# SegoleneMartin/transductive-CLIP

Hardware: AMD Instinct MI355X
Metric: transductive tasks/sec (75-query EM-Dirichlet) (higher is better)
Workload: dtype f32

## Files before the change

### transductive-clip_amd/csrc/tclip_device.h

```cpp
#pragma once
#include <hip/hip_runtime.h>

#include "tclip_math.h"
#include "tclip_rsqrt14_table_dev.h"

namespace tclip {

constexpr int kGroup = 32;
constexpr float kEpsF = 1e-15f;

template <int N>
__device__ __forceinline__ float dpp_row_shl(float v) {
    static_assert(N >= 1 && N <= 15, "row_shl");
    return __builtin_bit_cast(float, __builtin_amdgcn_update_dpp(0, __builtin_bit_cast(int, v), 0x100 + N, 0xf, 0xf, true));
}
__device__ __forceinline__ float ordered_sum8_lane0(float fin, float p0) {
    fin += p0;
    fin += dpp_row_shl<1>(p0);
    fin += dpp_row_shl<2>(p0);
    fin += dpp_row_shl<3>(p0);
    fin += dpp_row_shl<4>(p0);
    fin += dpp_row_shl<5>(p0);
    fin += dpp_row_shl<6>(p0);
    fin += dpp_row_shl<7>(p0);
// ... 254 lines not shown
    const float big = __builtin_fabsf(div_rn_inrange_f32(2.0f * t, a * a));
    const float curv = (a > 1e-11f) ? big : 1.6449340668482264f;
    float b = (psi1 - psi_s) - curv * a;
    b = b - y;
    const float delta = b * b + 4.0f * curv;
    const float nume = -b + sqrt_torch_inrange_dev(delta), deno = 2.0f * curv;
    return deno == 0.0f ? nume * __builtin_inff() : div_rn_inrange_f32(nume, deno);
}

__device__ __forceinline__ float mm_update(float a, float y, float psi_s, const LogTabEntry* tab) {
    float psi1, lg1;
    digamma_lgamma_xp1(a, tab, psi1, lg1);
    return mm_update_algebra(a, y, psi_s, psi1, lg1);
}

__device__ __noinline__ float mm_update_generic(float a, float y, float psi_s) {
    const float x1 = a + 1.0f;
    const float psi1 = digamma_f32(x1);
    const float lg1 = lgamma_f32(x1);
    float curv;
    if (a > 1e-11f) {
        const float t = (0.0f - lg1) + psi1 * a;
        curv = __builtin_fabsf((2.0f * t) / (a * a));
    } else {
        curv = 1.6449340668482264f;
    }
    float b = (psi1 - psi_s) - curv * a;
    b = b - y;
    const float delta = b * b + 4.0f * curv;
    return (-b + sqrt_torch_f32(delta)) / (2.0f * curv);
}

__device__ __forceinline__ void load_log_table(LogTabEntry* lds_tab) {
    if (threadIdx.x < 16) lds_tab[threadIdx.x] = kLogTab[threadIdx.x];
    __syncthreads();
}

}
```

### transductive-clip_amd/csrc/tclip_kernels.hip

```cpp
#include <hip/hip_runtime.h>
#include <stdint.h>
#include <stdio.h>
#include <stdlib.h>
#include <string.h>

#include <algorithm>
#include <mutex>
#include <utility>
#include <vector>

#include "../../include/tclip.h"
#include "tclip_device.h"
#include "tclip_pk.h"
#include "tclip_selftest_inputs.h"

namespace tclip {

constexpr int kG64MinK = 897;

__global__ void k_log_features(const float* __restrict__ x, float* __restrict__ out, size_t n, int32_t* __restrict__ nonfinite) {
    bool bad = false;
    for (size_t i = (size_t)blockIdx.x * blockDim.x + threadIdx.x; i < n; i += (size_t)gridDim.x * blockDim.x) {
        const float v = log_f32(x[i] + kEpsF);
        out[i] = v;
// ... 571 lines not shown
    }
    const float psi_s = digamma_pos_f32(s, tab);
    int n_big = 0;
#pragma unroll
    for (int e = 0; e < E; e++) {
        const float x1 = beta[e] + 1.0f;
        const bool big = x1 >= 2.3f;
        const unsigned long long m = __ballot(big);
        if (big) queue[n_big + lanes_below(m)] = x1;
        n_big += __popcll(m);
    }
    __builtin_amdgcn_wave_barrier();
    const unsigned long long active = __ballot(true);
    const int rank = lanes_below(active), n_active = __popcll(active);
    for (int start = 0; start < n_big; start += n_active) {
        const int idx = start + rank;
        const float v = idx < n_big ? queue[idx] : 8.0f;
        const float r = lgamma_big_dense(v);
        if (idx < n_big) queue[idx] = r;
    }
    __builtin_amdgcn_wave_barrier();
    if (n_big == 0) mm_apply_updates_small<E, G>(beta, yv, K, lane, psi_s, tab, measure, num, den);
    else mm_apply_updates<E, G>(beta, yv, K, lane, psi_s, tab, queue, 0, measure, num, den);
    __builtin_amdgcn_wave_barrier();
}

constexpr int kProbeChunks = 2;
constexpr int kMaxCycle = 64;

constexpr int kMMWavesLarge = 3;
constexpr int kMMWavesSmall = 4;
template <int E, int G>
__global__ __launch_bounds__(256, (E > 16 ? kMMWavesLarge : kMMWavesSmall)) void k_mm_probe(MMArgs a) {
    __shared__ LogTabEntry tab[16];
    __shared__ double cyc[256 / G][kMaxCycle][2];
    __shared__ float lg_queue[4][64 * E];
    load_log_table(tab);
    float* queue = lg_queue[threadIdx.x >> 6];
    const int lane = threadIdx.x & (G - 1);
    const int group = threadIdx.x / G;
    const int groups_per_block = blockDim.x / G;
    const int n = *a.n_rows;
    const int K = a.K;
    for (int i = blockIdx.x * groups_per_block + group; i < n; i += gridDim.x * groups_per_block) {
        const int row = a.rows[i];
        if (a.stop[row / a.rows_per_batch]) continue;
        const int have = a.cache_len[row];
        if (have != a.chunk + 1) {
            if (a.next_rows && have < a.n_checks && lane == 0) a.next_rows[atomicAdd(a.next_count, 1)] = row;
            continue;
        }
        const float* ref = a.beta_dead + (size_t)row * K;
        float beta[E];
        RowY<E, G> yv;
        yv.load(nullptr, lane, K);
#pragma unroll
        for (int e = 0; e < E; e++) {
            const int d = elem_of<E, G>(e, lane);
            beta[e] = d < K ? ref[d] : 0.0f;
        }
        int period = 0;
        for (int j = 0; j < kMaxCycle && period == 0; j++) {
            double pn = 0.0, pd = 0.0;
            mm_iterate<E, G>(beta, yv, K, lane, tab, queue, true, pn, pd);
            pn = group_sum_f64_g<G>(pn);
            pd = group_sum_f64_g<G>(pd);
            if (lane == 0) { cyc[group][j][0] = pn; cyc[group][j][1] = pd; }
            bool same = true;
#pragma unroll
            for (int e = 0; e < E; e++) {
                const int d = elem_of<E, G>(e, lane);
                if (d < K) same = same && (beta[e] == ref[d]);
            }
            const unsigned long long bal = __ballot(same);
            constexpr unsigned long long kAll = G == 64 ? ~0ull : (1ull << (G & 63)) - 1ull;
            const unsigned long long mine = (bal >> ((threadIdx.x & 63) & ~(G - 1))) & kAll;
            if (mine == kAll) period = j + 1;
        }
        if (period && lane == 0) {
            for (int m = a.chunk + 1; m < a.n_checks; m++) {
                const int j = (50 * (m + 1) - (a.l1 + 1)) % period;
                double* c = a.cache + ((size_t)row * a.n_checks + m) * 2;
                c[0] = cyc[group][j][0];
                c[1] = cyc[group][j][1];
            }
            a.cache_len[row] = a.n_checks;
        }
        if (!period && a.next_rows && lane == 0) a.next_rows[atomicAdd(a.next_count, 1)] = row;
    }
}

constexpr int kDeadHead = 12;
static_assert(kDeadHead <= 18, "the last snapshot (32 iterations after the head) must lie at or before the first checkpoint (iteration 50)");
template <int E, int G>
__global__ __launch_bounds__(256, (E > 16 ? kMMWavesLarge : kMMWavesSmall)) void k_mm_probe_head(MMArgs a) {
    __shared__ LogTabEntry tab[16];
    __shared__ double cyc[256 / G][kMaxCycle][2];
    __shared__ float lg_queue[4][64 * E];
    load_log_table(tab);
    float* queue = lg_queue[threadIdx.x >> 6];
    const int lane = threadIdx.x & (G - 1);
    const int group = threadIdx.x / G;
    const int groups_per_block = blockDim.x / G;
    const int n = *a.n_rows;
    const int K = a.K;
    for (int i = blockIdx.x * groups_per_block + group; i < n; i += gridDim.x * groups_per_block) {
        const int row = a.rows[i];
        if (a.stop[row / a.rows_per_batch]) continue;
        if (a.cache_len[row] != 0) {
            if (lane == 0) a.next_rows[atomicAdd(a.next_count, 1)] = row;
            continue;
        }
        float* ref = a.beta_dead + (size_t)row * K;
        float* ref8 = const_cast<float*>(a.y) + (size_t)row * K;
        float beta[E];
        RowY<E, G> yv;
        yv.load(nullptr, lane, K);
#pragma unroll
        for (int e = 0; e < E; e++) {
            const int d = elem_of<E, G>(e, lane);
            beta[e] = d < K ? ref[d] : 0.0f;
        }
        int period = 0, js = 0, base = 0;
        bool have8 = false;
        constexpr unsigned long long kAll = G == 64 ? ~0ull : (1ull << (G & 63)) - 1ull;
        const int shift = (threadIdx.x & 63) & ~(G - 1);
        for (int j = 0; j < kMaxCycle && period == 0; j++) {
            double pn = 0.0, pd = 0.0;
            mm_iterate<E, G>(beta, yv, K, lane, tab, queue, true, pn, pd);
// ... 121 lines not shown
        }
        __syncthreads();
        return;
    }
    for (int start = ((wave + turn) % W) * 64; start < n_big; start += 64 * W) {
        const int j = start + lane64;
        int at = j;
#pragma unroll
        for (int w = 1; w < W; w++) at += j >= before[w] ? 64 * E * R - (before[w] - before[w - 1]) : 0;
        const float v = j < n_big ? queue[at] : 8.0f;
        const float r = lgamma_big_dense(v);
        if (j < n_big) queue[at] = r;
    }
    if (wave == (W - (turn % W) + 1) % W && lane64 < kGroups * R)
        ctl->psi[turn & 1][lane64] = digamma_pos_f32(ctl->rowsum[turn & 1][lane64], tab);
    __syncthreads();
    if (base[R] == 0) {
#pragma unroll
        for (int r = 0; r < R; r++)
            if (active[r])
                mm_apply_updates_small<E, G>(beta[r], yv[r], K, lane, ctl->psi[turn & 1][r * kGroups + (threadIdx.x / G)], tab,
                                             measure, num[r], den[r]);
        return;
    }
#pragma unroll
    for (int r = 0; r < R; r++)
        if (active[r])
            mm_apply_updates<E, G>(beta[r], yv[r], K, lane, ctl->psi[turn & 1][r * kGroups + (threadIdx.x / G)], tab, slice, base[r],
                                   measure, num[r], den[r]);
}

template <int E, int W, bool kDead, int R, int G = kGroup, int KC = 0>
__global__ __launch_bounds__(64 * W, (E > 16 ? kMMWavesLarge : kMMWavesSmall)) void k_mm_live(MMArgs a) {
    __shared__ LogTabEntry tab[16];
    __shared__ float queue[64 * W * E * R];
    __shared__ QueueCtl ctl;
    if (threadIdx.x == 0) ctl.bad = 0;
    load_log_table(tab);
    const int lane = threadIdx.x & (G - 1);
    const int group = threadIdx.x / G;
    constexpr int kGroups = (64 / G) * W, kRows = kGroups * R;
    static_assert(kRows <= 64, "QueueCtl holds 64 row sums");
    int turn = 0;
    const int n = *a.n_rows;
    const int K = KC > 0 ? KC : a.K;
    for (int first = blockIdx.x * kRows; first < n; first += gridDim.x * kRows) {
        int row[R];
        bool active[R];
        bool any = false;
#pragma unroll
        for (int r = 0; r < R; r++) {
            const int i = first + r * kGroups + group;
            row[r] = i < n ? a.rows[i] : 0;
            if constexpr (G == 64) row[r] = __builtin_amdgcn_readfirstlane(row[r]);
            const bool running = i < n && !a.stop[row[r] / a.rows_per_batch];
            const int have = (kDead && running) ? a.cache_len[row[r]] : 0;
            active[r] = running && (!kDead || have == a.chunk);
            any = any || active[r];
            if (kDead && a.next_rows && running && have < a.n_checks && lane == 0)
                a.next_rows[atomicAdd(a.next_count, 1)] = row[r];
        }
        if (!__syncthreads_or(any)) continue;
        const float* src = (kDead && a.chunk > 0) ? a.beta_dead : a.alpha;
        float* dst = kDead ? a.beta_dead : a.alpha;
        float beta[R][E];
        RowY<E, G> yv[R];
        double num[R], den[R];
// ... 199 lines not shown
        uint32_t largest = 0u;
#pragma unroll
        for (int e = 0; e < E; e++) largest = max(largest, f32_bits(beta[e]));
        in_domain = in_domain & mm_fast_domain_of_max_bits(largest);
    }
    s = __shfl(s, 0, G);
    if (__builtin_expect(!__all(in_domain), 0)) {
        if (active) {
            const float psi_s = digamma_f32(s);
#pragma unroll
            for (int e = 0; e < E; e++) {
                const float nb = mm_update_generic(beta[e], yv.get(e), psi_s);
                const bool ok = elem_of<E, G>(e, lane) < K;
                if (measure && ok) {
                    const double df = (double)nb - (double)beta[e];
                    num += df * df;
                    den += (double)beta[e] * (double)beta[e];
                }
                beta[e] = ok ? nb : 0.0f;
            }
        }
        pl.valid = false;
        return;
    }
    constexpr int kFirstRagged = first_ragged_register<E, G, KC>();
    int32_t smallest = 0x7f800000;
#pragma unroll
    for (int e = 0; e < E; e++) {
        int32_t bits = (int32_t)f32_bits(beta[e]);
        if (e >= kFirstRagged) bits = elem_of<E, G>(e, lane) < K ? bits : 0x7f800000;
        smallest = bits < smallest ? bits : smallest;
    }
    const bool tiny = __builtin_amdgcn_ballot_w64(smallest <= (int32_t)0x2d2febffu) != 0ull;
    const float psi_s = digamma_pos_f32(s, tab);
    bool sort_now = !(keep_placement && pl.valid);
    for (;;) {
        if (sort_now) {
            split_place<E, G, KC>(beta, K, lane, my0, pl);
            pl.sorts++;
        } else split_scatter<E, G, KC>(beta, K, lane, my0, pl);
        const int nA = pl.nA, nB = pl.nB, nC = pl.nC;
        wave_lds_handoff();
        bool misplaced = false;
        int jA = 0;
        for (; jA + 64 < nA; jA += 128) {
            const int j = jA;
            const int i0 = j + lane64, i1 = min(i0 + 64, nA - 1);
            const f2 x{my0[i0], my0[i1]};
            if (!sort_now && __builtin_amdgcn_ballot_w64(!(fmaxf(x.x, x.y) < 2.3f)) != 0ull) { misplaced = true; break; }
            f2 xr = x, acc = pk(0.0f);
#pragma unroll
            for (int k = 0; k < 8; k++) {
                acc = acc - pk_rcp_rn(xr);
                xr = xr + pk(1.0f);
            }
            const f2 m{below10_f32(xr.x), below10_f32(xr.y)};
            acc = pk_fma(-m, pk_rcp_rn(xr), acc);
            xr = xr + m;
            const f2 psi = pk_digamma_after_rec(xr, acc, tab);
            const f2 lg = pk_lgamma_sleef_1_23(x);
            my0[i0] = lg.x;
            my1[i0] = psi.x;
            my0[i1] = lg.y;
            my1[i1] = psi.y;
        }
        for (; !misplaced && jA < nA; jA += 64) {
            const int i = min(jA + lane64, nA - 1);
            const float x = my0[i];
            if (!sort_now && __builtin_amdgcn_ballot_w64(!(x < 2.3f)) != 0ull) { misplaced = true; break; }
            float xr = x, acc = 0.0f;
#pragma unroll
            for (int k = 0; k < 8; k++) {
                acc = acc - rcp_rn_f32(xr);
                xr = xr + 1.0f;
            }
            const float m = below10_f32(xr);
            acc = __builtin_fmaf(-m, rcp_rn_f32(xr), acc);
            xr = xr + m;
            const float psi = digamma_after_rec_ge10<false>(xr, acc, tab);
            bool sure;
            float lg = lgamma_sleef_1_23_f64(x, sure);
            if (__builtin_expect(__builtin_amdgcn_ballot_w64(!sure) != 0ull, 0)) lg = sure ? lg : lgamma_sleef_05_23(x);
            my0[i] = lg;
            my1[i] = psi;
        }
        auto pass_b = [&](int i) -> bool {
            const float x = my0[i];
            if (!sort_now && __builtin_amdgcn_ballot_w64(!(x >= 2.3f)) != 0ull) return true;
            float xr = x, acc = 0.0f;
#pragma unroll
            for (int k = 0; k < 8; k++) {
                const float m = below10_f32(xr);
                acc = __builtin_fmaf(-m, rcp_rn_f32(xr), acc);
                xr += m;
            }
            const float psi = digamma_after_rec_ge10<false>(xr, acc, tab);
            const float lg = lgamma_big_dense(x);
            my0[i] = lg;
            my1[i] = psi;
            return false;
        };
        const int tB = nB & 63, tC = nC & 63;
        const bool merged = tB > 0 && tC > 0 && tB + tC <= 64;
        const int endB = merged ? nB - tB : nB, endC = merged ? nC - tC : nC;
        for (int j = 0; !misplaced && j < endB; j += 64) misplaced = pass_b(nA + min(j + lane64, endB - 1));
        if (merged && !misplaced) {
            const int l = min(lane64, tB + tC - 1);
            misplaced = pass_b(l < tB ? nA + endB + l : nA + nB + endC + (l - tB));
        }
        for (int j = 0; !misplaced && j < endC; j += 64) {
            const int i = nA + nB + min(j + lane64, endC - 1);
            const float x = my0[i];
            if (!sort_now && __builtin_amdgcn_ballot_w64(!(x >= 10.0f)) != 0ull) { misplaced = true; break; }
            const float psi = digamma_after_rec_ge10<true>(x, 0.0f, tab);
            const float lg = lgamma_gt7_dense(x);
            my0[i] = lg;
            my1[i] = psi;
        }
        if (!misplaced) break;
        sort_now = true;
        wave_lds_handoff();
    }
    pl.valid = true;
    wave_lds_handoff();
    if (__builtin_expect(measure, 0)) {
        if (tiny) split_apply_updates<E, G, true, true>(beta, yv, K, lane, psi_s, my0, my1, pl.slot, num, den);
        else split_apply_updates<E, G, false, true>(beta, yv, K, lane, psi_s, my0, my1, pl.slot, num, den);
    } else if (__builtin_expect(tiny, 0)) split_apply_updates<E, G, true, false>(beta, yv, K, lane, psi_s, my0, my1, pl.slot, num, den);
    else split_apply_updates<E, G, false, false>(beta, yv, K, lane, psi_s, my0, my1, pl.slot, num, den);
    wave_lds_handoff();
}

template <int E, int G, int KC = 0>
__global__ __launch_bounds__(64, (E > 16 ? kMMWavesLarge : kMMWavesSmall)) void k_mm_split(MMArgs a) {
    static_assert(E <= kSplitMaxE, "LDS: two words per element");
    __shared__ LogTabEntry tab[16];
    __shared__ float plane0[64 * E];
    __shared__ float plane1[64 * E];
    load_log_table(tab);
    const int lane = threadIdx.x & (G - 1);
    const int group = threadIdx.x / G;
    constexpr int kRows = 64 / G;
    const int n = *a.n_rows;
    const int K = KC > 0 ? KC : a.K;
    for (int first = blockIdx.x * kRows; first < n; first += gridDim.x * kRows) {
        const int i = first + group;
        int row = i < n ? a.rows[i] : 0;
        if constexpr (G == 64) row = __builtin_amdgcn_readfirstlane(row);
        const bool active = i < n && !a.stop[row / a.rows_per_batch];
        if (!__any(active)) continue;
        float beta[E];
        RowY<E, G, kSplitYRegsMaxE> yv;
        double num = 0.0, den = 0.0;
        yv.load(a.y + (size_t)row * K, lane, K);
#pragma unroll
        for (int e = 0; e < E; e++) {
            const int d = elem_of<E, G>(e, lane);
            beta[e] = (active && d < K) ? a.alpha[(size_t)row * K + d] : 0.0f;
        }
        SplitPlacement<E> pl;
        pl.valid = false;
        pl.sorts = 0;
        for (int l = a.l0; l <= a.l1; l++)
            mm_iterate_wave_split<E, G, KC>(beta, yv, K, lane, active, tab, plane0, plane1, a.has_check && l == a.l1, num, den, pl,
                                            a.keep_placement != 0);
        if (a.work_counter && (threadIdx.x & 63) == 0) {
            atomicAdd(a.work_counter + 1, (unsigned long long)(a.l1 - a.l0 + 1));
            atomicAdd(a.work_counter + 2, (unsigned long long)pl.sorts);
        }
// ... 989 lines not shown
                blk = 0.0f;
#pragma unroll 8
                for (int j = 0; j < kFrontBlock; j++) blk = __builtin_fmaf(emb[d + j], tr[d + j], blk);
                acc += blk;
            }
            blk = 0.0f;
            for (; d < D; d++) blk = __builtin_fmaf(emb[d], tr[d], blk);
        }
        if (full < D) acc += blk;
        if (kScaleAfter) acc = temperature * acc;
        logit[k] = acc;
        mx = acc > mx ? acc : mx;
    }
    for (int m = 32; m >= 1; m >>= 1) { const float o = __shfl_xor(mx, m, 64); mx = o > mx ? o : mx; }
    __syncthreads();
    if (lane == 0) red[4 + wave] = mx;
    __syncthreads();
    mx = fmaxf(fmaxf(red[4], red[5]), fmaxf(red[6], red[7]));
    float sum = 0.0f;
    for (int k = tid; k < K; k += blockDim.x) {
        const float e = exp_f32_sleef(logit[k] - mx);
        logit[k] = e;
        sum += e;
    }
    for (int m = 32; m >= 1; m >>= 1) sum += __shfl_xor(sum, m, 64);
    __syncthreads();
    if (lane == 0) red[wave] = sum;
    __syncthreads();
    const float inv = 1.0f / (red[0] + red[1] + red[2] + red[3]);
    for (int k = tid; k < K; k += blockDim.x) z[(size_t)n * K + k] = logit[k] * inv;
}

__global__ void k_selftest(unsigned long long* out) {
    __shared__ LogTabEntry tab[16];
    load_log_table(tab);
    const uint32_t tid = blockIdx.x * blockDim.x + threadIdx.x, nth = gridDim.x * blockDim.x;
    unsigned long long b0 = 0, b1 = 0, b2 = 0, b3 = 0, b4 = 0, b5 = 0;
    for (uint32_t m = tid; m < (1u << 23); m += nth) {
        const float x = bits_f32(0x3f800000u | m);
        b0 += rcp_rn_f32(x) != 1.0f / x;
        b5 += rcp_rn2_f32(x) != 1.0f / x;
        const float xs = x * 0x1p-60f, xl = x * 0x1p60f;
        b0 += rcp_rn_f32(xs) != 1.0f / xs;
        b0 += rcp_rn_f32(xl) != 1.0f / xl;
    }
    for (uint32_t i = tid; i < (1u << 28); i += nth) {
        const float a = rand_float(i, 1u, -40, 81), b = rand_float(i, 2u, -40, 81);
        b1 += div_rn_inrange_f32(a, b) != a / b;
        b1 += div_rn_inrange_f32(-a, b) != (-a) / b;
    }
    for (uint32_t i = tid; i < (1u << 24); i += nth) {
        const float a = rand_float(i, 3u, -45, 70);
        float p, l;
        digamma_lgamma_xp1(a, tab, p, l);
        b2 += p != digamma_f32(a + 1.0f);
        b2 += digamma_pos_f32(a, tab) != digamma_f32(a);
        b3 += l != lgamma_f32(a + 1.0f);
        const uint32_t h = mix32(i * 7u + 3u);
        const float y = -0.001f - 40.0f * (float)(h & 0xffffu) / 65536.0f;
        const float ps = 0.5f + 14.0f * (float)(h >> 16) / 65536.0f;
        const float uf = mm_update(a, y, ps, tab), ug = mm_update_generic(a, y, ps);
        const bool differ = !(uf == ug || (uf != uf && ug != ug));
        b4 += differ;
        if (differ) { out[14] = f32_bits(a); out[15] = f32_bits(y); out[16] = f32_bits(ps); out[17] = f32_bits(uf); out[18] = f32_bits(ug); }
        const float a2 = rand_float(i, 4u, -12, 18);
        const f2 av{a, a2};
        const f2 lgb{a + 1.0f >= 2.3f ? lgamma_sleef_ge23<true>(a + 1.0f) : 0.0f,
// ... 1280 lines not shown
```

### transductive-clip_amd/csrc/tclip_math.h

```cpp
#pragma once
#include <stdint.h>

#include "tclip_rsqrt14_table.h"
#include "tclip_rcp14_log_table.h"

#if defined(__HIPCC__)
#define TCLIP_HD __host__ __device__ __forceinline__
#else
#define TCLIP_HD static inline
#endif

namespace tclip {

TCLIP_HD uint32_t f32_bits(float f) { return __builtin_bit_cast(uint32_t, f); }
TCLIP_HD float bits_f32(uint32_t u) { return __builtin_bit_cast(float, u); }
TCLIP_HD uint64_t f64_bits(double f) { return __builtin_bit_cast(uint64_t, f); }
TCLIP_HD double bits_f64(uint64_t u) { return __builtin_bit_cast(double, u); }

TCLIP_HD float rcp_rn_f32(float x) {
#if defined(__HIP_DEVICE_COMPILE__)
    const float r = __builtin_amdgcn_rcpf(x);
    const float e = __builtin_fmaf(-x, r, 1.0f);
    return __builtin_fmaf(e, r, r);
#else
// ... 1 lines not shown
#endif
}

TCLIP_HD float rcp_rn2_f32(float x) {
#if defined(__HIP_DEVICE_COMPILE__)
    float r = __builtin_amdgcn_rcpf(x);
    float e = __builtin_fmaf(-x, r, 1.0f);
    r = __builtin_fmaf(e, r, r);
    e = __builtin_fmaf(-x, r, 1.0f);
    return __builtin_fmaf(e, r, r);
#else
    return 1.0f / x;
#endif
}

TCLIP_HD float div_rn_inrange_f32(float a, float b) {
#if defined(__HIP_DEVICE_COMPILE__)
    const float r = rcp_rn_f32(b);
    const float q = a * r;
    const float rem = __builtin_fmaf(-b, q, a);
    return __builtin_fmaf(rem, r, q);
#else
    return a / b;
#endif
}

template <bool kFast>
TCLIP_HD float rcp_ieee(float x) {
    if (kFast) return rcp_rn_f32(x);
    return 1.0f / x;
}

struct LogTabEntry { double invc, logc; };
#define TCLIP_LOG_TABLE_INIT { \
    {0x1.661ec79f8f3bep+0, -0x1.57bf7808caadep-2}, {0x1.571ed4aaf883dp+0, -0x1.2bef0a7c06ddbp-2}, \
    {0x1.49539f0f010bp+0, -0x1.01eae7f513a67p-2},  {0x1.3c995b0b80385p+0, -0x1.b31d8a68224e9p-3}, \
    {0x1.30d190c8864a5p+0, -0x1.6574f0ac07758p-3}, {0x1.25e227b0b8eap+0, -0x1.1aa2bc79c81p-3},   \
    {0x1.1bb4a4a1a343fp+0, -0x1.a4e76ce8c0e5ep-4}, {0x1.12358f08ae5bap+0, -0x1.1973c5a611cccp-4}, \
    {0x1.0953f419900a7p+0, -0x1.252f438e10c1ep-5}, {0x1p+0, 0x0p+0},                             \
    {0x1.e608cfd9a47acp-1, 0x1.aa5aa5df25984p-5},  {0x1.ca4b31f026aap-1, 0x1.c5e53aa362eb4p-4},   \
    {0x1.b2036576afce6p-1, 0x1.526e57720db08p-3},  {0x1.9c2d163a1aa2dp-1, 0x1.bc2860d22477p-3},   \
    {0x1.886e6037841edp-1, 0x1.1058bc8a07ee1p-2},  {0x1.767dcf5534862p-1, 0x1.4043057b6ee09p-2}}

#if defined(__HIP_DEVICE_COMPILE__)
static __device__ __constant__ LogTabEntry kLogTab[16] = TCLIP_LOG_TABLE_INIT;
#else
static const LogTabEntry kLogTab[16] = TCLIP_LOG_TABLE_INIT;
#endif

constexpr double kLn2 = 0x1.62e42fefa39efp-1;

TCLIP_HD void log_reduce_tab(float x, const LogTabEntry* tab, double& r, double& y0) {
    const uint32_t ix = f32_bits(x);
    const uint32_t tmp = ix - 0x3f330000u;
    const int i = (tmp >> 19) & 15;
    const int k = (int32_t)tmp >> 23;
    const double z = (double)bits_f32(ix - (tmp & 0xff800000u));
    const LogTabEntry t = tab[i];
    r = __builtin_fma(z, t.invc, -1.0);
    y0 = t.logc + (double)k * kLn2;
}

TCLIP_HD float logf_glibc_tab(float x, const LogTabEntry* tab) {
    if (f32_bits(x) == 0x3f800000u) return 0.0f;
    double r, y0;
    log_reduce_tab(x, tab, r, y0);
    const double r2 = r * r;
    double y = __builtin_fma(0x1.5575b0be00b6ap-2, r, -0x1.ffffef20a4123p-2);
    y = __builtin_fma(-0x1.00ea348b88334p-2, r2, y);
    y = __builtin_fma(y, r2, y0 + r);
    return (float)y;
}
TCLIP_HD float logf_glibc(float x) { return logf_glibc_tab(x, kLogTab); }

#define TCLIP_SLN_T1 {0.0f, -0x1.f800000000000p-6f, -0x1.f0c0000000000p-5f, -0x1.6f00000000000p-4f, -0x1.e280000000000p-4f, -0x1.2950000000000p-3f, -0x1.5ff0000000000p-3f, -0x1.9520000000000p-3f, -0x1.c900000000000p-3f, -0x1.fb90000000000p-3f, -0x1.1678000000000p-2f, -0x1.2e90000000000p-2f, -0x1.4618000000000p-2f, -0x1.5d18000000000p-2f, -0x1.73a0000000000p-2f, -0x1.89a0000000000p-2f, -0x1.9f30000000000p-2f, -0x1.b450000000000p-2f, -0x1.c900000000000p-2f, -0x1.dd48000000000p-2f, -0x1.f128000000000p-2f, -0x1.0254000000000p-1f, -0x1.0be8000000000p-1f, -0x1.154c000000000p-1f, -0x1.1e84000000000p-1f, -0x1.2794000000000p-1f, -0x1.307c000000000p-1f, -0x1.3940000000000p-1f, -0x1.41d8000000000p-1f, -0x1.4a50000000000p-1f, -0x1.52a4000000000p-1f, -0x1.5ad4000000000p-1f}
#define TCLIP_SLN_T2 {0.0f, -0x1.4d873c0000000p-17f, 0x1.cf3fee0000000p-17f, -0x1.a515ca0000000p-17f, 0x1.f123aa0000000p-17f, -0x1.4be0800000000p-17f, -0x1.83853c0000000p-18f, -0x1.6a73d20000000p-17f, 0x1.070cac0000000p-20f, -0x1.86d5e40000000p-19f, 0x1.1aa2a20000000p-17f, 0x1.d451ee0000000p-18f, -0x1.78438c0000000p-19f, -0x1.edfac00000000p-17f, 0x1.404a220000000p-17f, -0x1.9c360a0000000p-17f, -0x1.1f65fc0000000p-17f, 0x1.10866e0000000p-19f, 0x1.070cac0000000p-19f, 0x1.5fb3e40000000p-18f, -0x1.ebf5e00000000p-19f, -0x1.2a5a5e0000000p-17f, 0x1.a37b5a0000000p-18f, -0x1.e97a6a0000000p-20f, -0x1.f5e7040000000p-17f, -0x1.e1289c0000000p-17f, -0x1.7334f20000000p-17f, 0x1.f2ca9e0000000p-17f, -0x1.fd08ce0000000p-18f, 0x1.e893f00000000p-19f, 0x1.2d9a440000000p-17f, -0x1.30d67c0000000p-23f}
struct Rcp14Buckets { uint32_t e[64]; };
constexpr Rcp14Buckets make_rcp14_buckets() {
    constexpr uint32_t start[TCLIP_RCP14_LOG_STEPS] = TCLIP_RCP14_LOG_START;
    Rcp14Buckets b{};
    for (uint32_t q = 0; q < 64; q++) {
        const uint32_t lo = q << 17, hi = lo + (1u << 17);
        uint32_t base = 0, thr = 1u << 23;
        for (int t = 1; t < TCLIP_RCP14_LOG_STEPS; t++) {
            if (start[t] <= lo) base++;
            else if (start[t] < hi) thr = start[t];
        }
        b.e[q] = (thr << 6) | base;
    }
    return b;
}
constexpr bool rcp14_table_is_regular() {
    constexpr uint32_t start[TCLIP_RCP14_LOG_STEPS] = TCLIP_RCP14_LOG_START;
// ... 482 lines not shown
}
TCLIP_HD float digamma_rec_acc_ge23(float x1) {
    float x = x1, acc = 0.0f;
#if defined(__HIP_DEVICE_COMPILE__)
#pragma unroll
#endif
    for (int j = 0; j < 8; j++) {
        const float m = below10_f32(x);
        acc = __builtin_fmaf(-m, rcp_rn_f32(x), acc);
        x += m;
    }
    return acc;
}
TCLIP_HD float digamma_rec_x_loop(float x1) {
    float x = x1;
    for (int j = 0; j < 9; j++) x += below10_f32(x);
    return x;
}
TCLIP_HD float digamma_rec_x(float x1) {
    const float f = x1 - __builtin_floorf(x1);
    const float r8 = ((f + 2.0f) + 2.0f) + 4.0f;
#if defined(__HIP_DEVICE_COMPILE__)
    const float up = __builtin_amdgcn_fmed3f(__builtin_fmaf(r8, 0x1p20f, 1.0f - 9.0f * 0x1p20f), 0.0f, 1.0f);
#else
    const float up = r8 == 9.0f ? 1.0f : 0.0f;
#endif
    const float small_x = (r8 + 2.0f) - up;
    return x1 < 10.0f ? small_x : x1;
}
TCLIP_HD float digamma_after_rec(float x, float acc, const LogTabEntry* tab) {
    const float series = digamma_series<true>(x, acc, tab);
    return (x == 10.0f) ? acc + 2.25175258906672110764f : series;
}
template <bool kNoAcc>
TCLIP_HD float digamma_after_rec_ge10(float x, float acc, const LogTabEntry* tab) {
    const float z = rcp_ieee<true>(x * x);
    float p = 8.33333333333333333333E-2f;
    p = __builtin_fmaf(p, z, -2.10927960927960927961E-2f);
    p = __builtin_fmaf(p, z, 7.57575757575757575758E-3f);
    p = __builtin_fmaf(p, z, -4.16666666666666666667E-3f);
    p = __builtin_fmaf(p, z, 3.96825396825396825397E-3f);
    p = __builtin_fmaf(p, z, -8.33333333333333333333E-3f);
    p = __builtin_fmaf(p, z, 8.33333333333333333333E-2f);
    const float y = z * p;
    double r, y0;
    log_reduce_tab(x, tab, r, y0);
    const double r2 = r * r;
    double l = __builtin_fma(0x1.5575b0be00b6ap-2, r, -0x1.ffffef20a4123p-2);
    l = __builtin_fma(-0x1.00ea348b88334p-2, r2, l);
    l = __builtin_fma(l, r2, y0 + r);
    const float lg = (float)l;
    const float series = ((kNoAcc ? lg : acc + lg) - 0.5f * rcp_ieee<true>(x)) - y;
    const float at10 = kNoAcc ? 2.25175258906672110764f : acc + 2.25175258906672110764f;
#if defined(__HIP_DEVICE_COMPILE__)
    if (__builtin_expect(__builtin_amdgcn_ballot_w64(x == 10.0f) == 0ull, 1)) return series;
#endif
    return (x == 10.0f) ? at10 : series;
}

TCLIP_HD void digamma_lgamma_xp1(float a, const LogTabEntry* tab, float& psi1, float& lg1) {
    psi1 = digamma_xp1(a, tab);
    const float x1 = a + 1.0f;
    const bool lo = x1 < 2.3f;
    const float small_x = lgamma_sleef_05_23(lo ? x1 : 2.0f);
    const float large_x = lgamma_sleef_ge23<true>(lo ? 8.0f : x1);
    lg1 = lo ? small_x : large_x;
}

}
```

### transductive-clip_amd/csrc/tclip_pk.h

```cpp
#pragma once
#include "tclip_device.h"

namespace tclip {

typedef float f2 __attribute__((ext_vector_type(2)));
typedef int i2 __attribute__((ext_vector_type(2)));

__device__ __forceinline__ f2 pk(float v) { return f2{v, v}; }
__device__ __forceinline__ f2 pk_fma(f2 a, f2 b, f2 c) { return __builtin_elementwise_fma(a, b, c); }
__device__ __forceinline__ f2 pk_sel(i2 m, f2 a, f2 b) { return m ? a : b; }
__device__ __forceinline__ f2 pk_sel(i2 m, float a, float b) { return m ? pk(a) : pk(b); }

__device__ __forceinline__ f2 pk_rcp_rn(f2 x) {
    f2 r{__builtin_amdgcn_rcpf(x.x), __builtin_amdgcn_rcpf(x.y)};
    const f2 e = pk_fma(-x, r, pk(1.0f));
    return pk_fma(e, r, r);
}

__device__ __forceinline__ f2 pk_div_rn(f2 a, f2 b) {
    const f2 r = pk_rcp_rn(b);
    const f2 q = a * r;
    const f2 rem = pk_fma(-b, q, a);
    return pk_fma(rem, r, q);
}

__device__ __forceinline__ f2 pk_div_rn_negden(f2 a, f2 nb) {
    const f2 r0{__builtin_amdgcn_rcpf(-nb.x), __builtin_amdgcn_rcpf(-nb.y)};
    const f2 r = pk_fma(pk_fma(nb, r0, pk(1.0f)), r0, r0);
    const f2 q = a * r;
    return pk_fma(pk_fma(nb, q, a), r, q);
}

__device__ __forceinline__ f2 pk_logf_glibc_ne1(f2 x, const LogTabEntry* tab) {
    const uint32_t ix0 = f32_bits(x.x), ix1 = f32_bits(x.y);
    const uint32_t tmp0 = ix0 - 0x3f330000u, tmp1 = ix1 - 0x3f330000u;
    const LogTabEntry e0 = tab[(tmp0 >> 19) & 15], e1 = tab[(tmp1 >> 19) & 15];
    const double z0 = (double)bits_f32(ix0 - (tmp0 & 0xff800000u)), z1 = (double)bits_f32(ix1 - (tmp1 & 0xff800000u));
    const double r0 = __builtin_fma(z0, e0.invc, -1.0), r1 = __builtin_fma(z1, e1.invc, -1.0);
    const double y00 = e0.logc + (double)((int32_t)tmp0 >> 23) * kLn2, y01 = e1.logc + (double)((int32_t)tmp1 >> 23) * kLn2;
    const double q0 = r0 * r0, q1 = r1 * r1;
    double y0 = __builtin_fma(0x1.5575b0be00b6ap-2, r0, -0x1.ffffef20a4123p-2);
    double y1 = __builtin_fma(0x1.5575b0be00b6ap-2, r1, -0x1.ffffef20a4123p-2);
    y0 = __builtin_fma(-0x1.00ea348b88334p-2, q0, y0);
    y1 = __builtin_fma(-0x1.00ea348b88334p-2, q1, y1);
    y0 = __builtin_fma(y0, q0, y00 + r0);
    y1 = __builtin_fma(y1, q1, y01 + r1);
    return f2{(float)y0, (float)y1};
}

__device__ __forceinline__ f2 pk_digamma_xp1(f2 a, const LogTabEntry* tab) {
    f2 x = a + pk(1.0f), acc = pk(0.0f);
#pragma unroll
    for (int j = 0; j < 9; j++) {
        const f2 m{below10_f32(x.x), below10_f32(x.y)};
        const f2 r = pk_rcp_rn(x);
        acc = pk_fma(-m, r, acc);
        x = x + m;
    }
    const f2 z = pk_rcp_rn(x * x);
    f2 p = pk(8.33333333333333333333E-2f);
    p = pk_fma(p, z, pk(-2.10927960927960927961E-2f));
    p = pk_fma(p, z, pk(7.57575757575757575758E-3f));
    p = pk_fma(p, z, pk(-4.16666666666666666667E-3f));
    p = pk_fma(p, z, pk(3.96825396825396825397E-3f));
    p = pk_fma(p, z, pk(-8.33333333333333333333E-3f));
    p = pk_fma(p, z, pk(8.33333333333333333333E-2f));
    const f2 y = z * p;
    const f2 lg = pk_logf_glibc_ne1(x, tab);
    const f2 series = ((acc + lg) - pk(0.5f) * pk_rcp_rn(x)) - y;
    return pk_sel(x == pk(10.0f), acc + pk(2.25175258906672110764f), series);
}

__device__ __forceinline__ f2 pk_digamma_rec_acc(f2 x1) {
    f2 x = x1, acc = pk(0.0f);
#pragma unroll
    for (int j = 0; j < 9; j++) {
        const f2 m{below10_f32(x.x), below10_f32(x.y)};
        const f2 r = pk_rcp_rn(x);
        acc = pk_fma(-m, r, acc);
        x = x + m;
    }
    return acc;
}
__device__ __forceinline__ f2 pk_digamma_rec_acc_lt23(f2 x1) {
    f2 x = x1, acc = pk(0.0f);
#pragma unroll
    for (int j = 0; j < 8; j++) {
        acc = acc - pk_rcp_rn(x);
        x = x + pk(1.0f);
    }
    const f2 m{below10_f32(x.x), below10_f32(x.y)};
    return pk_fma(-m, pk_rcp_rn(x), acc);
}
__device__ __forceinline__ f2 pk_digamma_rec_x(f2 x1) {
    const f2 f = x1 - __builtin_elementwise_floor(x1);
    const f2 r8 = ((f + pk(2.0f)) + pk(2.0f)) + pk(4.0f);
    const f2 up{__builtin_amdgcn_fmed3f(__builtin_fmaf(r8.x, 0x1p20f, 1.0f - 9.0f * 0x1p20f), 0.0f, 1.0f),
                __builtin_amdgcn_fmed3f(__builtin_fmaf(r8.y, 0x1p20f, 1.0f - 9.0f * 0x1p20f), 0.0f, 1.0f)};
    const f2 small_x = (r8 + pk(2.0f)) - up;
    return pk_sel(x1 < pk(10.0f), small_x, x1);
}
__device__ __forceinline__ f2 pk_digamma_after_rec(f2 x, f2 acc, const LogTabEntry* tab) {
    const f2 z = pk_rcp_rn(x * x);
    f2 p = pk(8.33333333333333333333E-2f);
    p = pk_fma(p, z, pk(-2.10927960927960927961E-2f));
    p = pk_fma(p, z, pk(7.57575757575757575758E-3f));
    p = pk_fma(p, z, pk(-4.16666666666666666667E-3f));
    p = pk_fma(p, z, pk(3.96825396825396825397E-3f));
    p = pk_fma(p, z, pk(-8.33333333333333333333E-3f));
    p = pk_fma(p, z, pk(8.33333333333333333333E-2f));
    const f2 y = z * p;
    const f2 lg = pk_logf_glibc_ne1(x, tab);
    const f2 series = ((acc + lg) - pk(0.5f) * pk_rcp_rn(x)) - y;
    return pk_sel(x == pk(10.0f), acc + pk(2.25175258906672110764f), series);
}

struct P2 { f2 x, y; };
__device__ __forceinline__ P2 pk_df_add2_f2_f(P2 a, f2 b) {
    const f2 s = a.x + b, v = s - a.x;
    const f2 t = (a.x - (s - v)) + (b - v);
    return P2{s, t + a.y};
}
__device__ __forceinline__ P2 pk_df_mul_f_f(f2 a, f2 b) {
    const f2 s = a * b;
    return P2{s, pk_fma(a, b, -s)};
}
__device__ __forceinline__ P2 pk_df_mul_f2_f(P2 a, f2 b) {
    const f2 s = a.x * b;
    return P2{s, pk_fma(a.y, b, pk_fma(a.x, b, -s))};
}

__device__ __forceinline__ f2 pk_lgamma_sleef_05_23(f2 x) {
    const i2 o0 = x <= pk(1.2f);
    const P2 d = pk_df_add2_f2_f(P2{x, pk(0.0f)}, pk_sel(o0, -1.0f, -2.0f));
    const f2 t = d.x + d.y;
    f2 u = pk_sel(o0, +0.9435157776e+0f, +0.1102489550e-3f);
    u = pk_fma(u, t, pk_sel(o0, +0.8670063615e+0f, +0.8160019934e-4f));
    u = pk_fma(u, t, pk_sel(o0, +0.4826702476e+0f, +0.1528468856e-3f));
    u = pk_fma(u, t, pk_sel(o0, -0.8855129778e-1f, -0.2355068718e-3f));
    u = pk_fma(u, t, pk_sel(o0, +0.1013825238e+0f, +0.4962242092e-3f));
    u = pk_fma(u, t, pk_sel(o0, -0.1493408978e+0f, -0.1193488017e-2f));
    u = pk_fma(u, t, pk_sel(o0, +0.1697509140e+0f, +0.2891599433e-2f));
    u = pk_fma(u, t, pk_sel(o0, -0.2072454542e+0f, -0.7385451812e-2f));
    u = pk_fma(u, t, pk_sel(o0, +0.2705872357e+0f, +0.2058077045e-1f));
    P2 z = pk_df_add2_f2_f(pk_df_mul_f_f(u, t), pk_sel(o0, -0.400686534596170958447352690395e+0f, -0.673523028297382446749257758235e-1f));
// ... 81 lines not shown
    else st.curv = bigv;
    st.b = (d - st.curv * a) - y;
    st.delta = pk_fma(pk(4.0f), st.curv, st.b * st.b);
    st.t0 = rsqrt14_entry(f32_bits(st.delta.x));
    st.t1 = rsqrt14_entry(f32_bits(st.delta.y));
    return st;
}
template <bool kTiny>
__device__ __forceinline__ PkUpdateStage pk_mm_update_stage1_given(f2 a, f2 y, float psi_s, float psi10, float psi11, float lg10, float lg11) {
    const float m0 = psi10 * a.x, m1 = psi11 * a.y;
    return pk_mm_update_stage1_core<kTiny>(a, y, m0 - lg10, m1 - lg11, f2{psi10 - psi_s, psi11 - psi_s});
}
__device__ __forceinline__ PkUpdateStage pk_mm_update_stage1(f2 a, f2 y, f2 psi_s, f2 lg_big, const LogTabEntry* tab) {
    const f2 x1 = a + pk(1.0f);
    const i2 big = x1 >= pk(2.3f);
    const f2 lg_small = pk_lgamma_sleef_1_23(pk_sel(big, pk(2.0f), x1));
    const f2 psi1 = pk_digamma_xp1(a, tab);
    const f2 lg1 = pk_sel(big, lg_big, lg_small);
    const f2 t = pk_t_of(lg1, psi1 * a);
    return pk_mm_update_stage1_core<true>(a, y, t.x, t.y, psi1 - psi_s);
}
__device__ __forceinline__ PkUpdateStage pk_mm_update_stage1_small(f2 a, f2 y, f2 psi_s, const LogTabEntry* tab) {
    const f2 x1 = a + pk(1.0f);
    const f2 lg1 = pk_lgamma_sleef_1_23(x1);
    f2 xr = x1, acc = pk(0.0f);
#pragma unroll
    for (int k = 0; k < 8; k++) {
        acc = acc - pk_rcp_rn(xr);
        xr = xr + pk(1.0f);
    }
    const f2 m{below10_f32(xr.x), below10_f32(xr.y)};
    acc = pk_fma(-m, pk_rcp_rn(xr), acc);
    xr = xr + m;
    const f2 psi1 = pk_digamma_after_rec(xr, acc, tab);
    const f2 t = pk_t_of(lg1, psi1 * a);
    return pk_mm_update_stage1_core<true>(a, y, t.x, t.y, psi1 - psi_s);
}
__device__ __forceinline__ f2 pk_mm_update_stage2(const PkUpdateStage& st) {
    const f2 yr{rsqrt14_from_entry(f32_bits(st.delta.x), st.t0), rsqrt14_from_entry(f32_bits(st.delta.y), st.t1)};
    const f2 s = st.delta * yr;
    const f2 root = pk_fma(pk_fma(-s, s, st.delta), pk(0.5f) * yr, s);
    const f2 nume = -st.b + root, deno = pk(2.0f) * st.curv;
    return pk_update_quotient(nume, deno);
}

__device__ __forceinline__ f2 pk_mm_update(f2 a, f2 y, f2 psi_s, f2 lg_big, const LogTabEntry* tab) {
    return pk_mm_update_stage2(pk_mm_update_stage1(a, y, psi_s, lg_big, tab));
}

}
```

Baseline: 162.0.

## Specialize log reduction for [10,16) and piggyback row-sum digamma on batched slot

```diff
diff --git a/transductive-clip_amd/csrc/tclip_device.h b/transductive-clip_amd/csrc/tclip_device.h
--- a/transductive-clip_amd/csrc/tclip_device.h
+++ b/transductive-clip_amd/csrc/tclip_device.h
@@ -310,7 +310,7 @@
 }
 
 __device__ __forceinline__ void load_log_table(LogTabEntry* lds_tab) {
-    if (threadIdx.x < 16) lds_tab[threadIdx.x] = kLogTab[threadIdx.x];
+    if (threadIdx.x < kLogTabEntries) lds_tab[threadIdx.x] = kLogTab[threadIdx.x];
     __syncthreads();
 }
 
diff --git a/transductive-clip_amd/csrc/tclip_kernels.hip b/transductive-clip_amd/csrc/tclip_kernels.hip
--- a/transductive-clip_amd/csrc/tclip_kernels.hip
+++ b/transductive-clip_amd/csrc/tclip_kernels.hip
@@ -627,7 +627,7 @@
 constexpr int kMMWavesSmall = 4;
 template <int E, int G>
 __global__ __launch_bounds__(256, (E > 16 ? kMMWavesLarge : kMMWavesSmall)) void k_mm_probe(MMArgs a) {
-    __shared__ LogTabEntry tab[16];
+    __shared__ LogTabEntry tab[kLogTabEntries];
     __shared__ double cyc[256 / G][kMaxCycle][2];
     __shared__ float lg_queue[4][64 * E];
     load_log_table(tab);
@@ -689,7 +689,7 @@
 static_assert(kDeadHead <= 18, "the last snapshot (32 iterations after the head) must lie at or before the first checkpoint (iteration 50)");
 template <int E, int G>
 __global__ __launch_bounds__(256, (E > 16 ? kMMWavesLarge : kMMWavesSmall)) void k_mm_probe_head(MMArgs a) {
-    __shared__ LogTabEntry tab[16];
+    __shared__ LogTabEntry tab[kLogTabEntries];
     __shared__ double cyc[256 / G][kMaxCycle][2];
     __shared__ float lg_queue[4][64 * E];
     load_log_table(tab);
@@ -877,7 +877,7 @@
 
 template <int E, int W, bool kDead, int R, int G = kGroup, int KC = 0>
 __global__ __launch_bounds__(64 * W, (E > 16 ? kMMWavesLarge : kMMWavesSmall)) void k_mm_live(MMArgs a) {
-    __shared__ LogTabEntry tab[16];
+    __shared__ LogTabEntry tab[kLogTabEntries];
     __shared__ float queue[64 * W * E * R];
     __shared__ QueueCtl ctl;
     if (threadIdx.x == 0) ctl.bad = 0;
@@ -1143,14 +1143,26 @@
         smallest = bits < smallest ? bits : smallest;
     }
     const bool tiny = __builtin_amdgcn_ballot_w64(smallest <= (int32_t)0x2d2febffu) != 0ull;
-    const float psi_s = digamma_pos_f32(s, tab);
+    constexpr int kRowsW = 64 / G;
+    const bool sums_ge10 = __builtin_amdgcn_ballot_w64(!(s >= 10.0f)) == 0ull;
+    bool rode = false;
     bool sort_now = !(keep_placement && pl.valid);
     for (;;) {
         if (sort_now) {
             split_place<E, G, KC>(beta, K, lane, my0, pl);
             pl.sorts++;
         } else split_scatter<E, G, KC>(beta, K, lane, my0, pl);
-        const int nA = pl.nA, nB = pl.nB, nC = pl.nC;
+        const int nA = pl.nA, nB = pl.nB;
+        int nC = pl.nC;
+        {
+            const int tB0 = nB & 63, tC0 = nC & 63;
+            const bool merged0 = tB0 > 0 && tC0 > 0 && tB0 + tC0 <= 64;
+            rode = sums_ge10 && tC0 > 0 && tC0 + kRowsW <= 64 && (!merged0 || tB0 + tC0 + kRowsW <= 64) && nA + nB + nC + kRowsW <= 64 * E;
+            if (rode) {
+                if (lane == 0) my0[nA + nB + nC + lane64 / G] = s;
+                nC += kRowsW;
+            }
+        }
         wave_lds_handoff();
         bool misplaced = false;
         int jA = 0;
@@ -1168,7 +1180,7 @@
             const f2 m{below10_f32(xr.x), below10_f32(xr.y)};
             acc = pk_fma(-m, pk_rcp_rn(xr), acc);
             xr = xr + m;
-            const f2 psi = pk_digamma_after_rec(xr, acc, tab);
+            const f2 psi = pk_digamma_after_rec<true>(xr, acc, tab);
             const f2 lg = pk_lgamma_sleef_1_23(x);
             my0[i0] = lg.x;
             my1[i0] = psi.x;
@@ -1188,7 +1200,7 @@
             const float m = below10_f32(xr);
             acc = __builtin_fmaf(-m, rcp_rn_f32(xr), acc);
             xr = xr + m;
-            const float psi = digamma_after_rec_ge10<false>(xr, acc, tab);
+            const float psi = digamma_after_rec_ge10<false, true>(xr, acc, tab);
             bool sure;
             float lg = lgamma_sleef_1_23_f64(x, sure);
             if (__builtin_expect(__builtin_amdgcn_ballot_w64(!sure) != 0ull, 0)) lg = sure ? lg : lgamma_sleef_05_23(x);
@@ -1234,6 +1246,7 @@
     }
     pl.valid = true;
     wave_lds_handoff();
+    const float psi_s = rode ? my1[pl.nA + pl.nB + pl.nC + lane64 / G] : digamma_pos_f32(s, tab);
     if (__builtin_expect(measure, 0)) {
         if (tiny) split_apply_updates<E, G, true, true>(beta, yv, K, lane, psi_s, my0, my1, pl.slot, num, den);
         else split_apply_updates<E, G, false, true>(beta, yv, K, lane, psi_s, my0, my1, pl.slot, num, den);
@@ -1245,7 +1258,7 @@
 template <int E, int G, int KC = 0>
 __global__ __launch_bounds__(64, (E > 16 ? kMMWavesLarge : kMMWavesSmall)) void k_mm_split(MMArgs a) {
     static_assert(E <= kSplitMaxE, "LDS: two words per element");
-    __shared__ LogTabEntry tab[16];
+    __shared__ LogTabEntry tab[kLogTabEntries];
     __shared__ float plane0[64 * E];
     __shared__ float plane1[64 * E];
     load_log_table(tab);
@@ -2301,7 +2314,7 @@
 }
 
 __global__ void k_selftest(unsigned long long* out) {
-    __shared__ LogTabEntry tab[16];
+    __shared__ LogTabEntry tab[kLogTabEntries];
     load_log_table(tab);
     const uint32_t tid = blockIdx.x * blockDim.x + threadIdx.x, nth = gridDim.x * blockDim.x;
     unsigned long long b0 = 0, b1 = 0, b2 = 0, b3 = 0, b4 = 0, b5 = 0;
diff --git a/transductive-clip_amd/csrc/tclip_math.h b/transductive-clip_amd/csrc/tclip_math.h
--- a/transductive-clip_amd/csrc/tclip_math.h
+++ b/transductive-clip_amd/csrc/tclip_math.h
@@ -57,23 +57,27 @@
 }
 
 struct LogTabEntry { double invc, logc; };
-#define TCLIP_LOG_TABLE_INIT { \
-    {0x1.661ec79f8f3bep+0, -0x1.57bf7808caadep-2}, {0x1.571ed4aaf883dp+0, -0x1.2bef0a7c06ddbp-2}, \
-    {0x1.49539f0f010bp+0, -0x1.01eae7f513a67p-2},  {0x1.3c995b0b80385p+0, -0x1.b31d8a68224e9p-3}, \
-    {0x1.30d190c8864a5p+0, -0x1.6574f0ac07758p-3}, {0x1.25e227b0b8eap+0, -0x1.1aa2bc79c81p-3},   \
-    {0x1.1bb4a4a1a343fp+0, -0x1.a4e76ce8c0e5ep-4}, {0x1.12358f08ae5bap+0, -0x1.1973c5a611cccp-4}, \
-    {0x1.0953f419900a7p+0, -0x1.252f438e10c1ep-5}, {0x1p+0, 0x0p+0},                             \
-    {0x1.e608cfd9a47acp-1, 0x1.aa5aa5df25984p-5},  {0x1.ca4b31f026aap-1, 0x1.c5e53aa362eb4p-4},   \
-    {0x1.b2036576afce6p-1, 0x1.526e57720db08p-3},  {0x1.9c2d163a1aa2dp-1, 0x1.bc2860d22477p-3},   \
-    {0x1.886e6037841edp-1, 0x1.1058bc8a07ee1p-2},  {0x1.767dcf5534862p-1, 0x1.4043057b6ee09p-2}}
-
-#if defined(__HIP_DEVICE_COMPILE__)
-static __device__ __constant__ LogTabEntry kLogTab[16] = TCLIP_LOG_TABLE_INIT;
-#else
-static const LogTabEntry kLogTab[16] = TCLIP_LOG_TABLE_INIT;
-#endif
-
 constexpr double kLn2 = 0x1.62e42fefa39efp-1;
+constexpr double log_range_y0(double logc, int k) { return logc + (double)k * kLn2; }
+#define TCLIP_LOG_ENTRIES(X) \
+    X(0x1.661ec79f8f3bep+0, -0x1.57bf7808caadep-2, 4) X(0x1.571ed4aaf883dp+0, -0x1.2bef0a7c06ddbp-2, 4) \
+    X(0x1.49539f0f010bp+0, -0x1.01eae7f513a67p-2, 4)  X(0x1.3c995b0b80385p+0, -0x1.b31d8a68224e9p-3, 4) \
+    X(0x1.30d190c8864a5p+0, -0x1.6574f0ac07758p-3, 4) X(0x1.25e227b0b8eap+0, -0x1.1aa2bc79c81p-3, 4)   \
+    X(0x1.1bb4a4a1a343fp+0, -0x1.a4e76ce8c0e5ep-4, 4) X(0x1.12358f08ae5bap+0, -0x1.1973c5a611cccp-4, 4) \
+    X(0x1.0953f419900a7p+0, -0x1.252f438e10c1ep-5, 4) X(0x1p+0, 0x0p+0, 4)                             \
+    X(0x1.e608cfd9a47acp-1, 0x1.aa5aa5df25984p-5, 4)  X(0x1.ca4b31f026aap-1, 0x1.c5e53aa362eb4p-4, 4)   \
+    X(0x1.b2036576afce6p-1, 0x1.526e57720db08p-3, 4)  X(0x1.9c2d163a1aa2dp-1, 0x1.bc2860d22477p-3, 3)   \
+    X(0x1.886e6037841edp-1, 0x1.1058bc8a07ee1p-2, 3)  X(0x1.767dcf5534862p-1, 0x1.4043057b6ee09p-2, 3)
+#define TCLIP_LOG_BASE_ENTRY(invc, logc, k) {invc, logc},
+#define TCLIP_LOG_RANGE_ENTRY(invc, logc, k) {(invc) * (1.0 / (double)(1 << (k))), log_range_y0(logc, k)},
+#define TCLIP_LOG_TABLE_INIT { TCLIP_LOG_ENTRIES(TCLIP_LOG_BASE_ENTRY) TCLIP_LOG_ENTRIES(TCLIP_LOG_RANGE_ENTRY) }
+constexpr int kLogTabEntries = 32;
+
+#if defined(__HIP_DEVICE_COMPILE__)
+static __device__ __constant__ LogTabEntry kLogTab[kLogTabEntries] = TCLIP_LOG_TABLE_INIT;
+#else
+static const LogTabEntry kLogTab[kLogTabEntries] = TCLIP_LOG_TABLE_INIT;
+#endif
 
 TCLIP_HD void log_reduce_tab(float x, const LogTabEntry* tab, double& r, double& y0) {
     const uint32_t ix = f32_bits(x);
@@ -84,6 +88,12 @@
     const LogTabEntry t = tab[i];
     r = __builtin_fma(z, t.invc, -1.0);
     y0 = t.logc + (double)k * kLn2;
+}
+
+TCLIP_HD void log_reduce_10_16(float x, const LogTabEntry* tab, double& r, double& y0) {
+    const LogTabEntry t = tab[16 + (((f32_bits(x) - 0x3f330000u) >> 19) & 15)];
+    r = __builtin_fma((double)x, t.invc, -1.0);
+    y0 = t.logc;
 }
 
 TCLIP_HD float logf_glibc_tab(float x, const LogTabEntry* tab) {
@@ -632,7 +642,7 @@
     const float series = digamma_series<true>(x, acc, tab);
     return (x == 10.0f) ? acc + 2.25175258906672110764f : series;
 }
-template <bool kNoAcc>
+template <bool kNoAcc, bool kLt16 = false>
 TCLIP_HD float digamma_after_rec_ge10(float x, float acc, const LogTabEntry* tab) {
     const float z = rcp_ieee<true>(x * x);
     float p = 8.33333333333333333333E-2f;
@@ -644,7 +654,8 @@
     p = __builtin_fmaf(p, z, 8.33333333333333333333E-2f);
     const float y = z * p;
     double r, y0;
-    log_reduce_tab(x, tab, r, y0);
+    if (kLt16) log_reduce_10_16(x, tab, r, y0);
+    else log_reduce_tab(x, tab, r, y0);
     const double r2 = r * r;
     double l = __builtin_fma(0x1.5575b0be00b6ap-2, r, -0x1.ffffef20a4123p-2);
     l = __builtin_fma(-0x1.00ea348b88334p-2, r2, l);
diff --git a/transductive-clip_amd/csrc/tclip_pk.h b/transductive-clip_amd/csrc/tclip_pk.h
--- a/transductive-clip_amd/csrc/tclip_pk.h
+++ b/transductive-clip_amd/csrc/tclip_pk.h
@@ -47,6 +47,18 @@
     y1 = __builtin_fma(y1, q1, y01 + r1);
     return f2{(float)y0, (float)y1};
 }
+__device__ __forceinline__ f2 pk_logf_glibc_10_16(f2 x, const LogTabEntry* tab) {
+    const LogTabEntry e0 = tab[16 + (((f32_bits(x.x) - 0x3f330000u) >> 19) & 15)], e1 = tab[16 + (((f32_bits(x.y) - 0x3f330000u) >> 19) & 15)];
+    const double r0 = __builtin_fma((double)x.x, e0.invc, -1.0), r1 = __builtin_fma((double)x.y, e1.invc, -1.0);
+    const double q0 = r0 * r0, q1 = r1 * r1;
+    double y0 = __builtin_fma(0x1.5575b0be00b6ap-2, r0, -0x1.ffffef20a4123p-2);
+    double y1 = __builtin_fma(0x1.5575b0be00b6ap-2, r1, -0x1.ffffef20a4123p-2);
+    y0 = __builtin_fma(-0x1.00ea348b88334p-2, q0, y0);
+    y1 = __builtin_fma(-0x1.00ea348b88334p-2, q1, y1);
+    y0 = __builtin_fma(y0, q0, e0.logc + r0);
+    y1 = __builtin_fma(y1, q1, e1.logc + r1);
+    return f2{(float)y0, (float)y1};
+}
 
 __device__ __forceinline__ f2 pk_digamma_xp1(f2 a, const LogTabEntry* tab) {
     f2 x = a + pk(1.0f), acc = pk(0.0f);
@@ -100,6 +112,7 @@
     const f2 small_x = (r8 + pk(2.0f)) - up;
     return pk_sel(x1 < pk(10.0f), small_x, x1);
 }
+template <bool kLt16 = false>
 __device__ __forceinline__ f2 pk_digamma_after_rec(f2 x, f2 acc, const LogTabEntry* tab) {
     const f2 z = pk_rcp_rn(x * x);
     f2 p = pk(8.33333333333333333333E-2f);
@@ -110,7 +123,7 @@
     p = pk_fma(p, z, pk(-8.33333333333333333333E-3f));
     p = pk_fma(p, z, pk(8.33333333333333333333E-2f));
     const f2 y = z * p;
-    const f2 lg = pk_logf_glibc_ne1(x, tab);
+    const f2 lg = kLt16 ? pk_logf_glibc_10_16(x, tab) : pk_logf_glibc_ne1(x, tab);
     const f2 series = ((acc + lg) - pk(0.5f) * pk_rcp_rn(x)) - y;
     return pk_sel(x == pk(10.0f), acc + pk(2.25175258906672110764f), series);
 }
@@ -258,7 +271,7 @@
     const f2 m{below10_f32(xr.x), below10_f32(xr.y)};
     acc = pk_fma(-m, pk_rcp_rn(xr), acc);
     xr = xr + m;
-    const f2 psi1 = pk_digamma_after_rec(xr, acc, tab);
+    const f2 psi1 = pk_digamma_after_rec<true>(xr, acc, tab);
     const f2 t = pk_t_of(lg1, psi1 * a);
     return pk_mm_update_stage1_core<true>(a, y, t.x, t.y, psi1 - psi_s);
 }
```

Result: no change. 163.0 (median of 6 runs) (+0.6%).
